# tyshiwo1/Accelerating-T2I-AR-with-SJD

Hardware: AMD Instinct MI355X
Metric: accepted image-tokens/s (SJD, Lumina-mGPT-7B 768px); tokens_per_step = 1/steps-to-converge rate (higher is better)
Workload: dtype bf16; 1 GPU; Lumina-mGPT-7B 768x768, 1 prompt/GPU, draft window 16, CFG 3.0 (batch 2), top-k 2000, bf16, random-init synthetic weights (embed_token_scale=0.7); prompt_len=64, kv_len_start=401, kv_len_end=2064, lead_in_steps=131, prompts=1, parallelism=prompt-parallel x1

## Files before the change

accelerating-t2i-ar-with-sjd_amd/_lib.py:

```python
import ctypes
import os

MAX_WINDOW = 64
MAX_RANGES = 4
DTYPE_BF16, DTYPE_F16, DTYPE_F32 = 0, 1, 2
F1_POST_NORM = 0x100
F2_ROPE_TABLE = 0x200
F2_HEAD_PAD128 = 0x400
K1_HEAD_DIM_100 = 0x800
F2_ONE_HEAD = 0x1000
QKN_SHARDS_SHIFT = 16

_HERE = os.path.dirname(os.path.abspath(__file__))
SO_PATH = os.environ.get("SJD_HIP_LIB") or os.path.join(_HERE, "libsjd_hip.so")


class RowRule(ctypes.Structure):
    _fields_ = [("n_ranges", ctypes.c_int32), ("lo", ctypes.c_int32 * MAX_RANGES), ("hi", ctypes.c_int32 * MAX_RANGES),
                ("forced", ctypes.c_int32), ("top_k", ctypes.c_int32), ("top_p_thr", ctypes.c_float), ("temperature", ctypes.c_float)]


class IterParams(ctypes.Structure):
    _fields_ = [("n_rows", ctypes.c_int32), ("kv_len", ctypes.c_int32), ("use_cfg", ctypes.c_int32),
                ("scheme", ctypes.c_int32), ("n_fresh", ctypes.c_int32), ("batch_rows", ctypes.c_int32), ("iter_seq", ctypes.c_int32), ("philox_blocks", ctypes.c_int32),
                ("philox_seed", ctypes.c_uint64), ("philox_offset", ctypes.c_uint64 * 3),
                ("fresh_tok", ctypes.c_int64 * MAX_WINDOW), ("rules", RowRule * MAX_WINDOW),
                ("resid_rules", RowRule * MAX_WINDOW)]


class State(ctypes.Structure):
    _fields_ = [("m", ctypes.c_int32), ("rejected", ctypes.c_int32), ("n_prev", ctypes.c_int32),
                ("prob_buf", ctypes.c_int32), ("tokens", ctypes.c_int64 * MAX_WINDOW),
                ("win_tok", ctypes.c_int64 * MAX_WINDOW), ("q_src", ctypes.c_int32 * MAX_WINDOW), ("amax", ctypes.c_int64 * MAX_WINDOW)]


class RowNorm(ctypes.Structure):
    _fields_ = [("sumsq", ctypes.c_void_p), ("slices", ctypes.c_int32), ("hidden", ctypes.c_int32), ("eps", ctypes.c_float)]


class RawUnits(ctypes.Structure):
    _fields_ = [("records", ctypes.c_void_p), ("index", ctypes.c_void_p), ("n", ctypes.c_int32)]


class Slots(ctypes.Structure):
    _fields_ = [("n_slots", ctypes.c_int32), ("head_rows", ctypes.c_int32), ("params_stride", ctypes.c_int64), ("state_stride", ctypes.c_int64),
                ("probs_stride", ctypes.c_int64), ("zero_state_stride", ctypes.c_int64), ("scratch_stride", ctypes.c_int64),
                ("mirror_stride", ctypes.c_int64), ("dbg_stride", ctypes.c_int64)]


class HeadPartials(ctypes.Structure):
    _fields_ = [("part", ctypes.c_void_p), ("n_chunks", ctypes.c_int32), ("chunk_stride", ctypes.c_int64), ("row_stride", ctypes.c_int64),
                ("col0", ctypes.c_int32), ("n_cols", ctypes.c_int32), ("urow_off", ctypes.c_int32), ("round_dtype", ctypes.c_int32),
                ("row_sumsq", ctypes.c_void_p), ("slices", ctypes.c_int32), ("prows", ctypes.c_int32), ("inv_hidden", ctypes.c_float),
                ("eps", ctypes.c_float), ("dbg_c", ctypes.c_void_p), ("dbg_u", ctypes.c_void_p), ("zero_state", ctypes.c_void_p)]


class L2Head(ctypes.Structure):
    _fields_ = [("wz", ctypes.c_void_p), ("kind", ctypes.c_int32), ("gx", ctypes.c_int32), ("gy", ctypes.c_int32), ("waves", ctypes.c_int32),
                ("n_tiles", ctypes.c_int32), ("tile0", ctypes.c_int32), ("n_out", ctypes.c_int32), ("pairs_full", ctypes.c_int32),
                ("pairs_last", ctypes.c_int32), ("step_major", ctypes.c_int32), ("head_pairs", ctypes.c_int32)]


EXPORTS = ["sjd_version", "sjd_error_string", "sjd_reguess", "sjd_logits_to_probs_sample", "sjd_verify_accept",
           "sjd_kv_append", "sjd_attention_workspace_bytes", "sjd_draft_window_attention", "sjd_draft_window_attention_ex",
           "sjd_event_create", "sjd_event_destroy", "sjd_event_synchronize", "sjd_event_elapsed_ms",
           "sjd_add_rmsnorm", "sjd_qknorm_rope_append", "sjd_silu_mul", "sjd_gemm_num_chunks", "sjd_skinny_gemm",
           "sjd_kv_append_fp8", "sjd_draft_window_attention_fp8", "sjd_qknorm_rope_append_fp8",
           "sjd_residual_sumsq", "sjd_qknorm_rope_append_ex", "sjd_silu_mul_ex", "sjd_skinny_gemm_cols",
           "sjd_logits_to_probs_sample_part", "sjd_logits_to_probs_sample_ex", "sjd_reguess_ex",
           "sjd_verify_accept_ex", "sjd_upload_async", "sjd_stream_synchronize", "sjd_gateup_silu", "sjd_host_wait_u64",
           "sjd_philox_fill", "sjd_philox_offset_increment", "sjd_skinny_gemm_z", "sjd_gateup_silu_z",
           "sjd_draft_window_attention_colsplit", "sjd_draft_window_attention_fp8_colsplit",
           "sjd_head_combine",
           "sjd_reguess_slots", "sjd_logits_to_probs_sample_part_slots", "sjd_verify_accept_slots",
           "sjd_logits_to_probs_sample_part_slots_g", "sjd_head_combine_g"]
EXP_EXPORTS = ["sjd_weight_prefetch", "sjd_qkv_attention_fused", "sjd_qkv_attention_fused_split", "sjd_skinny_gemm_reduce", "sjd_reduce_timeouts",
               "sjd_draft_window_attention_merged", "sjd_draft_window_attention_fp8_merged", "sjd_mlp_pair_z", "sjd_mlp_pair_timeouts",
               "sjd_l2_head_gemm_z", "sjd_l2_head_gateup_z", "sjd_l2_head_bytes", "sjd_weight_prefetch_head", "sjd_debug_xcc_map", "sjd_residual_sumsq_pf",
               "sjd_skinny_gemm_engine_z", "sjd_engine_timeouts", "sjd_skinny_gemm_wide", "sjd_o_merge_prologue_probe", "sjd_skinny_gemm_z_wide"]
EXP_SO_PATH = os.environ.get("SJD_HIP_EXP_LIB") or os.path.join(_HERE, "libsjd_hip_exp.so")
# ... 120 lines not shown
```

accelerating-t2i-ar-with-sjd_amd/backbones.py:

```python
import math
from dataclasses import dataclass
from typing import Optional

import torch
import torch.nn as nn
import torch.nn.functional as F


import logging as _logging
import os as _os
_log = _logging.getLogger("sjd_amd.backbones")

_K1_FUSED_DEFAULT = _os.environ.get("SJD_K1_FUSED", "0") == "1"
_K1_FUSED_SPLIT_DEFAULT = _os.environ.get("SJD_K1_FUSED_SPLIT", "1") != "0"
_MLP_PAIR_DEFAULT = _os.environ.get("SJD_MLP_PAIR", "0") == "1"
_NAN_CHECK = _os.environ.get("SJD_NAN_CHECK", "0") == "1"


def _chk(tag, x, rows=None):
    if not _NAN_CHECK or x is None:
        return x
    t = x.data if hasattr(x, "n_chunks") else x
    v = t if rows is None else (t[:, :rows] if hasattr(x, "n_chunks") else t[:rows])
    if not torch.isfinite(v.float()).all():
# ... 614 lines not shown
        try:
            self.forward_window(tokens, positions, 0, key_start)
        finally:
            self.cache, attn.params, attn.regime = cache, saved[0], saved[1]
        scales = []
        for li in range(len(self.model.layers)):
            ka = float(tmp.k[li][:, :, :P].abs().amax().float())
            va = float(tmp.v[li][:, :, :P].abs().amax().float())
            scales.append((max(ka, 1e-6) * headroom / 448.0, max(va, 1e-6) * headroom / 448.0))
        attn.layer_scales = scales
        self.buffers_version = getattr(self, "buffers_version", 0) + 1
        return scales

    def _f2(self, qkv, li, qn, pos, B, n, params, kv_len, row_norm=None):
        ops, H, Hkv, D = self._ops, self.n_heads, self.n_kv_heads, self.head_dim
        return ops.qknorm_rope_append(qkv, self.cache.k[li], self.cache.v[li], *qn, self._inv_freq32, pos, B, n, H, Hkv, D, params,
                                      kv_len if params is None else 0, kv_scale=self.attn.scale_of(li) if hasattr(self.attn, "scale_of") else (1.0, 1.0),
                                      dtype=self.lm_head.weight.dtype, row_norm=row_norm, qk_shards=self.args.model_parallel_size)

    def _attention_block(self, qkv_part, li, qn, pos, B, n, params, kv_len, key_start, row_norm=None):
        ops, H, Hkv, D = self._ops, self.n_heads, self.n_kv_heads, self.head_dim
        ks_ok = isinstance(key_start, torch.Tensor) and key_start.is_cuda and key_start.dtype == torch.int32
        if getattr(self, "k1_fused", _K1_FUSED_DEFAULT) and ks_ok and not self.args.swin_norm and self.args.model_parallel_size == 1 and ops.fused_attention_ok(B, n, H, Hkv, D, self.cache.k.dtype):
            ns, ws = 1, None
            if getattr(self, "k1_fused_split", _K1_FUSED_SPLIT_DEFAULT):
                ns = self.attn._resolve_split(B, Hkv, n, H)
                ws = self.attn._workspace(B, H, n, D, self.cache.k.device) if ns > 1 else None
            return ops.qkv_attention_fused(qkv_part, self.cache.k[li], self.cache.v[li], *qn, self._inv_freq32, pos, B, n, H, D, params,
                                           kv_len if params is None else 0, key_start, row_norm=row_norm, dtype=self.lm_head.weight.dtype,
                                           n_split=ns, workspace=ws)
        q = self._f2(qkv_part, li, qn, pos, B, n, params, kv_len, row_norm=row_norm)
        return self.attn.attend(li, q, self.cache, kv_len, key_start)

    def _forward_window_g1_folded(self, tokens, positions, kv_len, key_start, cols=None, head_partials=False):
        ops, B, n = self._ops, tokens.shape[0], tokens.shape[1]
        T, eps, cfg = B * n, self.args.rms_norm_eps, self.G1_CFG
        self._prefetch_plan()
        g1 = lambda x_, name, N_, K_: self._g1(li, x_, name, N_, K_)
        H, Hkv, D, hid, inter = self.n_heads, self.n_kv_heads, self.head_dim, self.args.hidden_size, self.args.intermediate_size
        params = getattr(self.attn, "params", None)
        want_fused = getattr(self, "gateup_fused", _GATEUP_FUSED_DEFAULT)
        fuse_mlp = want_fused and (T <= 64 or want_fused == "tall") and not self._pf_on and ops.gateup_silu_ok(T, inter, hid, cfg["gate_up"][0],
                                                                                                                   isinstance(self._packed[0]["gate_up"], ops.PackedZ))
        red = getattr(self, "reduce_fused", _REDUCE_FUSED_DEFAULT) and not self._pf_on
        raw = lambda name: not isinstance(self._packed[0][name], ops.PackedZ)
        h_dev = self.lm_head.weight.device
        red_o = red and raw("o") and ops.skinny_gemm_reduce_ok(T, hid, H * D, cfg["o"][0], 8, h_dev)
        red_d = red and raw("down") and ops.skinny_gemm_reduce_ok(T, hid, inter, cfg["down"][0], 8, h_dev)
        pair_mlp = (getattr(self, "mlp_pair", _MLP_PAIR_DEFAULT) and fuse_mlp and not red_d and h_dev.type == "cuda" and
                    ops.mlp_pair_ok(T, inter, hid, self._packed[0]["gate_up"], self._packed[0]["down"], cfg["down"][0], cfg["down"][1], h_dev))
        h = self.model.embed_tokens(tokens).view(T, -1).contiguous()
        pos = positions.reshape(T).contiguous()
        delta, ss_next = None, None
        for li, layer in enumerate(self.model.layers):
            a = layer.self_attn
            rn = (ss_next if ss_next is not None else ops.residual_sumsq(h, delta), hid, eps)
            qn = (a.q_norm.weight, a.q_norm.bias, a.k_norm.weight, a.k_norm.bias) if self.args.qk_norm else (None,) * 4
            _chk(f"L{li} sumsq", rn[0][:, :T] if rn[0].dim() == 2 and rn[0].shape[1] >= T else rn[0])
            o = self._attention_block(_chk(f"L{li} qkv", g1(h, "qkv", (H + 2 * Hkv) * D, hid), T), li, qn, pos, B, n, params, kv_len, key_start, row_norm=rn)
            _chk(f"L{li} attention", o)
            if red_o:
                rn = (ops.skinny_gemm_reduce(o.view(T, H * D), self._packed[li]["o"], hid, H * D, cfg["o"][0], h, 8, cfg["o"][2]), hid, eps)
            else:
                rn = (ops.residual_sumsq(h, g1(o.view(T, H * D), "o", hid, H * D)), hid, eps)
            if pair_mlp:
                if getattr(self, "_pair_ready", None) is None or self._pair_ready.device != h.device:
                    self._pair_ready = torch.zeros(max(64, (inter + cfg["down"][0] - 1) // cfg["down"][0] + 1), dtype=torch.int32, device=h.device)
                _, delta = ops.mlp_pair(h, self._packed[li]["gate_up"], self._packed[li]["down"], inter, hid, cfg["down"][0], row_norm=rn,
                                        ready=self._pair_ready)
                ss_next = None
                continue
            if fuse_mlp:
                act = ops.gateup_silu(h, self._packed[li]["gate_up"], inter, hid, cfg["gate_up"][2], row_norm=rn)
            else:
                act = ops.silu_mul(g1(h, "gate_up", 2 * inter, hid), rows=T, dtype=h.dtype, row_norm=rn)
            _chk(f"L{li} act", act)
            if red_d:
                delta, ss_next = None, ops.skinny_gemm_reduce(act, self._packed[li]["down"], hid, inter, cfg["down"][0], h, 8, cfg["down"][2])
            else:
                delta, ss_next = g1(act, "down", hid, inter), None
            _chk(f"L{li} down", delta, T)
            _chk(f"L{li} h", h)
        self._prefetch_join()
        if head_partials and self._packed_head is not None:
            return self._head_partials(h, delta, cols, n, sumsq=ss_next)
        if ss_next is not None:
# ... 5 lines not shown
    def _forward_window_g1(self, tokens, positions, kv_len, key_start, cols=None):
        ops, B, n = self._ops, tokens.shape[0], tokens.shape[1]
        T, eps, cfg = B * n, self.args.rms_norm_eps, self.G1_CFG
        cap = 2560 if T <= 32 else 1 << 30
        if any(c[0] > cap for c in cfg.values()):
            raise ValueError(f"G1_CFG chunk sizes must be <= {cap} for a {T}-row window")
        g1 = lambda x_, name, N_, K_: ops.skinny_gemm(x_, self._packed[li][name], N_, K_, cfg[name][0], cfg[name][1], cfg[name][2])
        H, Hkv, D, hid, inter = self.n_heads, self.n_kv_heads, self.head_dim, self.args.hidden_size, self.args.intermediate_size
        params = getattr(self.attn, "params", None)
        h = self.model.embed_tokens(tokens).view(T, -1).contiguous()
        pos = positions.reshape(T).contiguous()
        delta = None
        swin = self.args.swin_norm
        for li, layer in enumerate(self.model.layers):
            a = layer.self_attn
            x = h if swin else ops.add_rmsnorm(h, delta, layer.input_layernorm.weight, eps)
            qkv = g1(x, "qkv", (H + 2 * Hkv) * D, hid)
            qn = (a.q_norm.weight, a.q_norm.bias, a.k_norm.weight, a.k_norm.bias) if self.args.qk_norm else (None,) * 4
            o = self._attention_block(qkv, li, qn, pos, B, n, params, kv_len, key_start)
            attn_out = g1(o.view(T, H * D), "o", hid, H * D)
            if swin:
                x = ops.add_rmsnorm_post(h, attn_out, layer.input_layernorm.weight, eps)
            else:
                x = ops.add_rmsnorm(h, attn_out, layer.post_attention_layernorm.weight, eps)
            gu = g1(x, "gate_up", 2 * inter, hid)
            act = ops.silu_mul(gu, rows=T, dtype=h.dtype)
            delta = g1(act, "down", hid, inter)
            if swin:
                ops.add_rmsnorm_post(h, delta, layer.post_attention_layernorm.weight, eps)
                delta = None
        x = ops.add_rmsnorm(h, delta, self.model.norm.weight, eps)
        return _head_logits(self.lm_head, x, cols).view(B, n, -1)

    def _forward_window_fused(self, tokens, positions, kv_len, key_start, cols=None, head_partials=False):
        T_ = tokens.shape[0] * tokens.shape[1]
        if self._gemm == "sjd" and (T_ <= 64 or (T_ <= 128 and tokens.shape[1] <= 32) or
                                    (T_ <= 256 and tokens.shape[1] <= 32 and self._packed and not isinstance(self._packed[0]["qkv"], self._ops.PackedZ)
                                     and all(c[1] in self.G1_WIDE_TILES for c in self.G1_CFG.values()))):
            if self._fold_norm:
                return self._forward_window_g1_folded(tokens, positions, kv_len, key_start, cols, head_partials)
            return self._forward_window_g1(tokens, positions, kv_len, key_start, cols)
        ops, B, n = self._ops, tokens.shape[0], tokens.shape[1]
        T, eps = B * n, self.args.rms_norm_eps
        H, Hkv, D = self.n_heads, self.n_kv_heads, self.head_dim
        params = getattr(self.attn, "params", None)
        h = self.model.embed_tokens(tokens).view(T, -1).contiguous()
        pos = positions.reshape(T).contiguous()
        delta = None
        swin = self.args.swin_norm
        for li, layer in enumerate(self.model.layers):
            a = layer.self_attn
            qkv_w, gu_w = self._fused[li]
            x = h if swin else ops.add_rmsnorm(h, delta, layer.input_layernorm.weight, eps)
            qkv = F.linear(x, qkv_w)
            qn = (a.q_norm.weight, a.q_norm.bias, a.k_norm.weight, a.k_norm.bias) if self.args.qk_norm else (None,) * 4
            q = _chk(f"prefill L{li} q", self._f2(_chk(f"prefill L{li} qkv", qkv), li, qn, pos, B, n, params, kv_len))
            o = _chk(f"prefill L{li} attention", self.attn.attend(li, q, self.cache, kv_len, key_start))
            attn_out = F.linear(o.view(T, H * D), a.o_proj.weight)
            if swin:
                x = _chk(f"prefill L{li} norm1", ops.add_rmsnorm_post(h, attn_out, layer.input_layernorm.weight, eps))
                ops.add_rmsnorm_post(h, _chk(f"prefill L{li} mlp", F.linear(ops.silu_mul(F.linear(x, gu_w)), layer.mlp.down_proj.weight)),
                                     layer.post_attention_layernorm.weight, eps)
                continue
            x = _chk(f"prefill L{li} norm2", ops.add_rmsnorm(h, attn_out, layer.post_attention_layernorm.weight, eps))
            delta = _chk(f"prefill L{li} mlp", F.linear(ops.silu_mul(F.linear(x, gu_w)), layer.mlp.down_proj.weight))
        x = ops.add_rmsnorm(h, delta, self.model.norm.weight, eps)
        return _head_logits(self.lm_head, x, cols).view(B, n, -1)

    def forward_window(self, tokens, positions, kv_len, key_start, cols=None, head_partials=False):
        if getattr(self, "_ops", None) is not None:
            return self._forward_window_fused(tokens, positions, kv_len, key_start, cols, head_partials)
        B, n = tokens.shape
        h = self.model.embed_tokens(tokens)
        cos, sin = self._rope(positions, h.dtype)
        for li, layer in enumerate(self.model.layers):
            a = layer.self_attn
            x = h if self.args.swin_norm else layer.input_layernorm(h)
            q = a.q_proj(x).view(B, n, a.num_heads, a.head_dim)
            k = a.k_proj(x).view(B, n, a.num_kv, a.head_dim)
            v = a.v_proj(x).view(B, n, a.num_kv, a.head_dim)
            if self.args.qk_norm:
                q, k = a.q_norm(q), a.k_norm(k)
            q = q * cos + _rotate_half(q) * sin
            k = k * cos + _rotate_half(k) * sin
            o = self.attn(li, q, k, v, self.cache, kv_len, key_start)
            if self.args.swin_norm:
                h = h + layer.input_layernorm(a.o_proj(o.reshape(B, n, -1)))
                h = h + layer.post_attention_layernorm(layer.mlp(h))
                continue
            h = h + a.o_proj(o.reshape(B, n, -1))
            h = h + layer.mlp(layer.post_attention_layernorm(h))
        return _head_logits(self.lm_head, self.model.norm(h), cols)


LUMINA_7B = ChameleonArgs()
CHAMELEON_30B = ChameleonArgs(vocab_size=65536, hidden_size=8192, intermediate_size=22016, num_hidden_layers=48, num_attention_heads=64,
                              num_key_value_heads=8, model_parallel_size=4, swin_norm=True)
EMU3_8B = ChameleonArgs(vocab_size=184622, hidden_size=4096, intermediate_size=14336, num_hidden_layers=32,
                        num_attention_heads=32, num_key_value_heads=8, rms_norm_eps=1e-5, rope_theta=1000000.0,
                        qk_norm=False, max_position_embeddings=9216)
LLAMAGEN_B = LlamaGenArgs(dim=768, n_layer=12, n_head=12)
```

accelerating-t2i-ar-with-sjd_amd/csrc/sjd_sampling.hip:

```cpp
#include <hip/hip_runtime.h>
#include <math.h>
#include <type_traits>

#include "../../include/sjd_hip.h"
#include "sjd_device.h"
#include "sjd_philox.h"

#ifdef SJD_TRACE
__device__ unsigned long long g_k2_trace[64][16];
#define SJD_TRS(slot, i) do { if (threadIdx.x == 0) g_k2_trace[(slot) & 63][i] = wall_clock64(); } while (0)
extern "C" int sjd_debug_trace_k2(unsigned long long *host_out, int n)
{
    return hipMemcpyFromSymbol(host_out, HIP_SYMBOL(g_k2_trace), (size_t)n * 16 * sizeof(unsigned long long), 0, hipMemcpyDeviceToHost) == hipSuccess ? 0 : -1;
}
#else
#define SJD_TRS(slot, i) do { } while (0)
#endif

__device__ __forceinline__ void rule_window(const sjd_row_rule &r, int V, int &lo, int &hi)
{
    if (r.n_ranges == 0) { lo = 0; hi = V; return; }
    lo = V; hi = 0;
#pragma unroll
    for (int a = 0; a < SJD_MAX_RANGES; ++a)
        if (a < r.n_ranges) { lo = min(lo, r.lo[a]); hi = max(hi, r.hi[a]); }
    lo = max(lo, 0); hi = min(hi, V);
    if (hi < lo) hi = lo;
}

__device__ __forceinline__ bool rule_allows(const sjd_row_rule &r, int c)
{
    if (r.n_ranges == 0) return true;
    bool ok = false;
#pragma unroll
    for (int a = 0; a < SJD_MAX_RANGES; ++a) ok |= (a < r.n_ranges) && (c >= r.lo[a]) && (c < r.hi[a]);
    return ok;
}

static_assert(sizeof(sjd_row_rule) == 52 && sizeof(sjd_iter_params) == 64 + 8 * SJD_MAX_WINDOW + 2 * 52 * SJD_MAX_WINDOW, "sjd_iter_params layout is mirrored by ctypes (sjd_amd/_lib.py::IterParams)");
static_assert(sizeof(sjd_head_partials) == 96, "sjd_head_partials layout is mirrored by ctypes (sjd_amd/_lib.py::HeadPartials)");

__device__ __forceinline__ float k2_round16(float x, int dt)
{
    if (dt == SJD_DTYPE_BF16) {
        unsigned u = __float_as_uint(x);
        u += 0x7fffu + ((u >> 16) & 1u);
        return __uint_as_float(u & 0xffff0000u);
    }
    if (dt == SJD_DTYPE_F16) return (float)((_Float16)x);
    return x;
}

__device__ __forceinline__ float k2_row_scale(const sjd_head_partials &hp, int tok)
{
    if (!hp.row_sumsq) return 1.0f;
    float t = 0.f;
    for (int s0 = 0; s0 < hp.slices; s0 += 8) {
        float v[8];
#pragma unroll
        for (int q = 0; q < 8; ++q) v[q] = (s0 + q < hp.slices) ? hp.row_sumsq[(size_t)(s0 + q) * hp.prows + tok] : 0.f;
#pragma unroll
        for (int q = 0; q < 8; ++q) t += v[q];
    }
    return rsqrtf(t * hp.inv_hidden + hp.eps);
}

__device__ __forceinline__ void k2_row_scales(const sjd_head_partials &hp, int tok, float &rc, float &ru)
{
    if (!hp.row_sumsq) return;
    const bool two = hp.urow_off > 0;
    float t = 0.f, tu = 0.f;
    for (int s0 = 0; s0 < hp.slices; s0 += 8) {
// ... 683 lines not shown
                            const unsigned long long cand = pack_vi(dv / sjd_philox_exponential(ph_seed, ph_off2, ph_T2, (uint64_t)col), col);
                            best = cand > best ? cand : best;
                        }
                    } else {
                        SJD_FOR_OWNED_COLS_IN(wlo, whi, c0) {
#pragma unroll
                            for (int j = 0; j < 4; ++j) {
                                const int col = c0 + j;
                                if (col >= wlo && col < whi) {
                                    const float dv = scratch[col - sb] / S;
                                    if (dv > 0.0f) {
                                        const unsigned long long cand = pack_vi(dv / sjd_philox_exponential(ph_seed, ph_off2, ph_T2, (uint64_t)col), col);
                                        best = cand > best ? cand : best;
                                    }
                                }
                            }
                        }
                    }
                }
                SJD_TRS(32, 4);
                const int tok = block_argmax(best, sh);
                if (threadIdx.x == 0) state->tokens[row] = tok;
            }
            };
            if (res_lds) resample(std::true_type{}); else resample(std::false_type{});
        }
    }
    if (threadIdx.x == 0) { state->m = m; state->rejected = rejected ? (degenerate ? 2 : 1) : 0; state->n_prev = n; }
    SJD_TRS(32, 5);
    k4_mirror_state(state, host_mirror, params->iter_seq);
    SJD_TRS(32, 6);
}

template <bool SLOTS = false>
__global__ void k5_reguess(const sjd_iter_params *__restrict__ params, sjd_state *__restrict__ state,
                           int64_t *__restrict__ input_ids_out, int n_batch, int max_rows, const int64_t *__restrict__ pos_offset,
                           int64_t *__restrict__ positions_out, const sjd_slots sb)
{
    if constexpr (SLOTS) {
        const size_t s = blockIdx.x;
        params = reinterpret_cast<const sjd_iter_params *>(reinterpret_cast<const char *>(params) + s * (size_t)sb.params_stride);
        state = reinterpret_cast<sjd_state *>(reinterpret_cast<char *>(state) + s * (size_t)sb.state_stride);
        input_ids_out += s * (size_t)n_batch * (size_t)max_rows;
        if (pos_offset) pos_offset += s * (size_t)n_batch;
        if (positions_out) positions_out += s * (size_t)n_batch * (size_t)max_rows;
    }
    const int i = threadIdx.x;
    const int n = params->n_rows;
    const int m = state->m, n_prev = state->n_prev;
    int a = n_prev - m;
    if (a > n - 1) a = n - 1;
    if (a < 0) a = 0;
    int64_t tok = 0;
    int qs = -1;
    if (i < n) {
        if (i <= a) { tok = state->tokens[m - 1 + i]; qs = m - 1 + i; }
        else { tok = params->fresh_tok[i - 1 - a]; qs = -1; }
    }
    __syncthreads();
    if (i < max_rows) {
        if (i >= n) { tok = state->tokens[m - 1]; qs = -1; }
        state->win_tok[i] = tok;
        state->q_src[i] = qs;
        for (int b = 0; b < n_batch; ++b) input_ids_out[(size_t)b * max_rows + i] = tok;
        if (positions_out) {
            const int64_t base = (int64_t)params->kv_len + i;
            for (int b = 0; b < n_batch; ++b) positions_out[(size_t)b * max_rows + i] = base + (pos_offset ? pos_offset[b] : 0);
        }
    }
}

#define SJD_DRAW_LIST 2304
static int sjd_stage_lds_floats(long cols)
{
    const long cap = 150 * 1024 / 4;
    return (int)(cols < cap ? ((cols + 3) & ~3L) : cap);
}

extern "C" int sjd_reguess_ex(const sjd_iter_params *params, sjd_state *state, int64_t *input_ids_out, int n_batch, int max_rows,
                              const int64_t *pos_offset, int64_t *positions_out, void *stream)
{
    if (!params || !state || !input_ids_out || max_rows < 1 || max_rows > SJD_MAX_WINDOW || n_batch < 1) return SJD_ERR_BAD_ARG;
    hipLaunchKernelGGL(k5_reguess<false>, dim3(1), dim3(64), 0, (hipStream_t)stream, params, state, input_ids_out, n_batch, max_rows, pos_offset,
                       positions_out, sjd_slots{});
    return hipGetLastError() == hipSuccess ? SJD_OK : SJD_ERR_LAUNCH;
}

extern "C" int sjd_reguess(const sjd_iter_params *params, sjd_state *state, int64_t *input_ids_out, int n_batch,
                           int max_rows, void *stream)
{
    return sjd_reguess_ex(params, state, input_ids_out, n_batch, max_rows, nullptr, nullptr, stream);
}

extern "C" int sjd_logits_to_probs_sample_ex(const float *logits_c, const float *logits_u, int64_t row_stride, float guidance,
                                             int max_rows, int V, const sjd_iter_params *params, const float *noise,
                                             float *probs_out, int64_t *tokens_out, int64_t *amax_out, void *stream);

extern "C" int sjd_logits_to_probs_sample(const float *logits_c, const float *logits_u, int64_t row_stride, float guidance,
                                          int max_rows, int V, const sjd_iter_params *params, const float *noise,
                                          float *probs_out, int64_t *tokens_out, void *stream)
{
    return sjd_logits_to_probs_sample_ex(logits_c, logits_u, row_stride, guidance, max_rows, V, params, noise, probs_out, tokens_out, nullptr, stream);
// ... 51 lines not shown
    if (!guidance || ((uintptr_t)guidance & 3)) return SJD_ERR_BAD_ARG;
    return sjd_head_combine_launch(head, 0.0f, guidance, max_rows, V, params, z_out, stream);
}

extern "C" int sjd_verify_accept_ex(const sjd_iter_params *params, sjd_state *state, const float *probs, const float *prev_probs,
                                    const float *rs, const float *noise2, float *scratch, int max_rows, int V, sjd_state *host_mirror,
                                    void *stream)
{
    if (!params || !state || !probs || !prev_probs || !scratch || max_rows < 1 || max_rows > SJD_MAX_WINDOW || V < 1)
        return SJD_ERR_BAD_ARG;
    const int lds_floats = sjd_stage_lds_floats((long)V + 2 * SJD_DRAW_LIST);
    (void)hipFuncSetAttribute((const void *)k4_verify_accept<false>, hipFuncAttributeMaxDynamicSharedMemorySize, lds_floats * 4);
    hipLaunchKernelGGL(k4_verify_accept<false>, dim3(1), dim3(SJD_TPB), (size_t)lds_floats * 4, (hipStream_t)stream, params, state, probs, prev_probs, rs,
                       noise2, scratch, V, host_mirror, lds_floats, sjd_slots{});
    return hipGetLastError() == hipSuccess ? SJD_OK : SJD_ERR_LAUNCH;
}

extern "C" int sjd_verify_accept(const sjd_iter_params *params, sjd_state *state, const float *probs, const float *prev_probs,
                                 const float *rs, const float *noise2, float *scratch, int max_rows, int V, void *stream)
{
    return sjd_verify_accept_ex(params, state, probs, prev_probs, rs, noise2, scratch, max_rows, V, nullptr, stream);
}

static bool sjd_slots_ok(const sjd_slots *sl)
{
    return sl && sl->n_slots >= 1 && sl->n_slots <= 65535 && sl->params_stride >= (int64_t)sizeof(sjd_iter_params) && (sl->params_stride % 8) == 0 &&
           sl->state_stride >= (int64_t)sizeof(sjd_state) && (sl->state_stride % 8) == 0;
}

extern "C" int sjd_reguess_slots(const sjd_iter_params *params0, sjd_state *state0, int64_t *input_ids_out, int n_batch, int max_rows,
                                 const int64_t *pos_offset, int64_t *positions_out, const sjd_slots *slots, void *stream)
{
    if (!params0 || !state0 || !input_ids_out || max_rows < 1 || max_rows > SJD_MAX_WINDOW || n_batch < 1 || !sjd_slots_ok(slots)) return SJD_ERR_BAD_ARG;
    hipLaunchKernelGGL(k5_reguess<true>, dim3(slots->n_slots), dim3(64), 0, (hipStream_t)stream, params0, state0, input_ids_out, n_batch, max_rows,
                       pos_offset, positions_out, *slots);
    return hipGetLastError() == hipSuccess ? SJD_OK : SJD_ERR_LAUNCH;
}

static int sjd_k2_slots_launch(const sjd_head_partials *head, float guidance, const float *guidance_slots, int max_rows, int V,
                               const sjd_iter_params *params0, float *probs_out0, int64_t *tokens_out0, int64_t *amax_out0, const sjd_slots *slots,
                               void *stream)
{
    if (!head || !head->part || head->n_chunks < 1 || head->n_cols < 1 || head->col0 < 0 || head->row_stride < head->n_cols) return SJD_ERR_BAD_ARG;
    if (!params0 || !probs_out0 || !tokens_out0 || max_rows < 1 || max_rows > SJD_MAX_WINDOW || V < 1) return SJD_ERR_BAD_ARG;
    if (head->row_sumsq && (head->slices < 1 || head->prows < 1)) return SJD_ERR_BAD_ARG;
    if (!sjd_slots_ok(slots) || slots->head_rows < max_rows || slots->probs_stride < (int64_t)max_rows * V) return SJD_ERR_BAD_ARG;
    if (head->zero_state && slots->zero_state_stride < 2 * (int64_t)max_rows) return SJD_ERR_BAD_ARG;
    if ((head->dbg_c || head->dbg_u) && slots->dbg_stride < (int64_t)max_rows * V) return SJD_ERR_BAD_ARG;
    const int lds_floats = sjd_stage_lds_floats((long)head->n_cols + 8 + 2 * SJD_DRAW_LIST);
    (void)hipFuncSetAttribute((const void *)k2_logits_to_probs_sample<true, true>, hipFuncAttributeMaxDynamicSharedMemorySize, lds_floats * 4);
    hipLaunchKernelGGL((k2_logits_to_probs_sample<true, true>), dim3(max_rows, slots->n_slots), dim3(SJD_TPB), (size_t)lds_floats * 4, (hipStream_t)stream,
                       (const float *)nullptr, (const float *)nullptr, (long)0, guidance, V, params0, (const float *)nullptr, probs_out0, tokens_out0, *head,
                       amax_out0, lds_floats, *slots, guidance_slots);
    return hipGetLastError() == hipSuccess ? SJD_OK : SJD_ERR_LAUNCH;
}

extern "C" int sjd_logits_to_probs_sample_part_slots(const sjd_head_partials *head, float guidance, int max_rows, int V, const sjd_iter_params *params0,
                                                     float *probs_out0, int64_t *tokens_out0, int64_t *amax_out0, const sjd_slots *slots, void *stream)
{
    return sjd_k2_slots_launch(head, guidance, nullptr, max_rows, V, params0, probs_out0, tokens_out0, amax_out0, slots, stream);
}

extern "C" int sjd_logits_to_probs_sample_part_slots_g(const sjd_head_partials *head, const float *guidance, int max_rows, int V,
                                                       const sjd_iter_params *params0, float *probs_out0, int64_t *tokens_out0, int64_t *amax_out0,
                                                       const sjd_slots *slots, void *stream)
{
// ... 37 lines not shown
```

accelerating-t2i-ar-with-sjd_amd/engine.py:

```python
import contextlib
import ctypes
import gc
import os
import random
import time
import warnings
from dataclasses import dataclass, field
from typing import List, Optional

import numpy as np
import torch

from . import _lib as L
from . import ops
from .grammar import spatial_fresh_tokens


_MIRROR_STREAM_WAIT = os.environ.get("SJD_MIRROR_SPIN", "0") != "1"
_TWO_STAGE = os.environ.get("SJD_TWO_STAGE", "0") == "1"


@dataclass
class SJDConfig:
    jacobi_loop_interval_l: int = 1
# ... 147 lines not shown
        p = self.params.view
        p.n_rows, p.kv_len, p.use_cfg, p.scheme, p.n_fresh = n, kv_len, int(use_cfg), scheme, len(fresh)
        self._seq = (self._seq % 0x7FFFFFF0) + 1
        p.iter_seq = self._seq
        if philox is None:
            p.philox_blocks = 0
        else:
            p.philox_blocks, p.philox_seed = philox[0], philox[1]
            p.philox_offset[0], p.philox_offset[1], p.philox_offset[2] = philox[2], philox[3], philox[4]
        if fresh:
            p.fresh_tok[:len(fresh)] = fresh
        self._write_rules(L.IterParams.rules.offset, rules)
        if resid:
            self._write_rules(L.IterParams.resid_rules.offset, resid)
        self.params.upload(L.IterParams.resid_rules.offset if head_only else None)

    def _write_rules(self, offset, rules):
        key = tuple(map(id, rules))
        blk = self._rule_bytes.get(key)
        if blk is None:
            blk = b"".join(bytes(r) for r in rules)
            if len(self._rule_bytes) < 4096:
                self._rule_bytes[key] = blk
                self._rule_keep.append(list(rules))
        ctypes.memmove(self.params.host.data_ptr() + offset, blk, len(blk))

    def _upload_resid(self, resid):
        off = L.IterParams.resid_rules.offset
        self._write_rules(off, resid)
        L.check(L.load().sjd_upload_async(self.params.dev.data_ptr() + off, self.params.host.data_ptr() + off, self.params.nbytes - off,
                                          ops._stream()), "sjd_upload_async")

    def _forward_body(self, cols=None):
        ops.reguess(self.params, self.state, self.input_ids, pos_offset=self.pos_offset, positions_out=self.positions)
        positions = self.positions
        if self.head_partials:
            return self.backbone.forward_window(self.input_ids, positions, -1, self.key_start, cols=cols, head_partials=True)
        if cols is None:
            return self.backbone.forward_window(self.input_ids, positions, -1, self.key_start)
        return self.backbone.forward_window(self.input_ids, positions, -1, self.key_start, cols=cols)

    def _calibrate_fp8(self, tokens, positions, key_start):
        bb = self.backbone
        cache, attn = getattr(bb, "cache", None), getattr(bb, "attn", None)
        if (cache is None or cache.k.dtype != ops.FP8 or attn is None or getattr(attn, "layer_scales", 1) is not None
                or getattr(attn, "kv_scale", (1.0, 1.0)) != (1.0, 1.0) or not hasattr(bb, "calibrate_kv_scales")
                or os.environ.get("SJD_FP8_CALIBRATE", "1") == "0"):
            return
        bb.calibrate_kv_scales(tokens, positions, key_start)

    def _k2_out(self):
        return (self.amax_ptr, self.tokens_ptr) if getattr(self, "_greedy", False) else (self.tokens_ptr, self.amax_ptr)

    def _sample_body(self, cur, logits, cols=None):
        noise, rs, noise2 = (None, None, None) if self._philox else (self.noise, self.rs, self.noise2[0])
        if isinstance(logits, ops.HeadOut):
            dbg = None
            if self.hook is not None:
                if self._dbg is None:
                    self._dbg = torch.zeros(2, self.Lmax, self.V, dtype=torch.float32, device=self.device)
                dbg = self._dbg
                dbg.zero_()
            tok_out, amax_out = self._k2_out()
            ops.logits_to_probs_sample_part(logits, self._guidance, self.params, noise, self.probs[cur], tok_out, dbg=dbg,
                                            amax_out_ptr=amax_out, zero_state=self.zero_state[cur])
        else:
            lu = logits[1] if self.B > 1 else None
            tok_out, amax_out = self._k2_out()
# ... 316 lines not shown
```

accelerating-t2i-ar-with-sjd_amd/ops.py:

```python
import ctypes
import os

import torch

from . import _lib as L


def _stream():
    return ctypes.c_void_p(torch.cuda.current_stream().cuda_stream)


def _ptr(t):
    return ctypes.c_void_p(0 if t is None else t.data_ptr())


def _dtype_code(dt):
    if dt == torch.bfloat16:
        return L.DTYPE_BF16
    if dt == torch.float16:
        return L.DTYPE_F16
    if dt == torch.float32:
        return L.DTYPE_F32
    raise L.SjdLibraryError(f"SJD HIP kernels support bf16/fp16 KV and activations, got {dt}")

# ... 103 lines not shown
            st = self.nbytes + 8
            self._mirrors = torch.zeros(len(self.blobs) * st, dtype=torch.uint8, pin_memory=True)
            for i, b in enumerate(self.blobs):
                b._mirror = self._mirrors[i * st:(i + 1) * st]
        return ctypes.c_void_p(self._mirrors.data_ptr()), self.nbytes + 8

    def upload(self):
        L.check(L.load().sjd_upload_async(self.dev.data_ptr(), self.host.data_ptr(), self.host.numel(), _stream()), "sjd_upload_async")

    def download(self):
        self.host.copy_(self.dev)

    def wait_mirror(self):
        L.check(L.load().sjd_stream_synchronize(_stream()), "sjd_stream_synchronize")
        for b in self.blobs:
            if b._mirror is not None:
                b.collect_mirror()

    @property
    def ptr(self):
        return ctypes.c_void_p(self.dev.data_ptr())


def reguess(params: DeviceBlob, state: DeviceBlob, input_ids_out: torch.Tensor, pos_offset=None, positions_out=None):
    n_batch, max_rows = input_ids_out.shape
    assert input_ids_out.dtype == torch.int64 and input_ids_out.is_contiguous()
    if positions_out is None:
        L.check(L.load().sjd_reguess(params.ptr, state.ptr, _ptr(input_ids_out), n_batch, max_rows, _stream()), "sjd_reguess")
        return
    assert positions_out.dtype == torch.int64 and positions_out.is_contiguous() and tuple(positions_out.shape) == (n_batch, max_rows)
    assert pos_offset is None or (pos_offset.dtype == torch.int64 and pos_offset.is_contiguous() and pos_offset.numel() == n_batch)
    L.check(L.load().sjd_reguess_ex(params.ptr, state.ptr, _ptr(input_ids_out), n_batch, max_rows, _ptr(pos_offset) if pos_offset is not None else None,
                                   _ptr(positions_out), _stream()), "sjd_reguess_ex")


def logits_to_probs_sample(logits_c, logits_u, guidance, params: DeviceBlob, noise, probs_out, tokens_out_ptr, col0=0, amax_out_ptr=None):
    max_rows, V = probs_out.shape
    assert logits_c.dtype == torch.float32 and logits_c.stride(-1) == 1 and probs_out.is_contiguous()
    assert noise is None or (noise.dtype == torch.float32 and noise.is_contiguous() and noise.shape[-1] == V)
    if logits_u is not None:
        assert logits_u.stride(-2) == logits_c.stride(-2) and logits_u.stride(-1) == 1
    shift = lambda t: ctypes.c_void_p(0 if t is None else t.data_ptr() - 4 * int(col0))
    L.check(L.load().sjd_logits_to_probs_sample_ex(shift(logits_c), shift(logits_u), logits_c.stride(-2), float(guidance),
                                                  max_rows, V, params.ptr, _ptr(noise), _ptr(probs_out), tokens_out_ptr, amax_out_ptr,
                                                  _stream()), "sjd_logits_to_probs_sample")


def verify_accept(params: DeviceBlob, state: DeviceBlob, probs, prev_probs, rs, noise2, scratch, mirror=False):
    max_rows, V = probs.shape
    for t in (probs, prev_probs, rs, noise2, scratch):
        assert t is None or (t.dtype == torch.float32 and t.is_contiguous())
    L.check(L.load().sjd_verify_accept_ex(params.ptr, state.ptr, _ptr(probs), _ptr(prev_probs), _ptr(rs), _ptr(noise2),
                                         _ptr(scratch), max_rows, V, state.mirror_ptr if mirror else None, _stream()), "sjd_verify_accept")


def kv_append(k_new, v_new, k_cache, v_cache, params, kv_len):
    B, n, Hkv, D = k_new.shape
    assert k_new.is_contiguous() and v_new.is_contiguous() and k_cache.is_contiguous() and v_cache.is_contiguous()
    L.check(L.load().sjd_kv_append(_ptr(k_new), _ptr(v_new), _ptr(k_cache), _ptr(v_cache), B, n, Hkv, D,
                                  k_cache.shape[2], _dtype_code(k_new.dtype), params.ptr if params is not None else None,
                                  int(kv_len), _stream()), "sjd_kv_append")


FP8 = torch.float8_e4m3fn


# ... 847 lines not shown
```

include/sjd_hip.h:

```cpp
#ifndef SJD_HIP_H
#define SJD_HIP_H

#include <stdint.h>

#ifdef __cplusplus
extern "C" {
#endif

#define SJD_VERSION 104
#define SJD_MAX_WINDOW 64
#define SJD_MAX_RANGES 4

#define SJD_OK 0
#define SJD_ERR_BAD_ARG (-1)
#define SJD_ERR_UNSUPPORTED (-2)
#define SJD_ERR_LAUNCH (-3)

#define SJD_DTYPE_BF16 0
#define SJD_DTYPE_F16 1
#define SJD_DTYPE_F32 2

#define SJD_DTYPE_MASK 0xff
#define SJD_F1_POST_NORM 0x100
#define SJD_F2_ROPE_TABLE 0x200
// ... 77 lines not shown
                               int max_rows, int V, const sjd_iter_params *params, const float *noise,
                               float *probs_out, int64_t *tokens_out, void *stream);
int sjd_logits_to_probs_sample_ex(const float *logits_c, const float *logits_u, int64_t row_stride, float guidance,
                                  int max_rows, int V, const sjd_iter_params *params, const float *noise,
                                  float *probs_out, int64_t *tokens_out, int64_t *amax_out, void *stream);

typedef struct sjd_head_partials {
    const float *part;
    int32_t n_chunks;
    int64_t chunk_stride;
    int64_t row_stride;
    int32_t col0, n_cols;
    int32_t urow_off;
    int32_t round_dtype;
    const float *row_sumsq;
    int32_t slices, prows;
    float inv_hidden, eps;
    float *dbg_c, *dbg_u;
    int32_t *zero_state;
} sjd_head_partials;
int sjd_logits_to_probs_sample_part(const sjd_head_partials *head , float guidance,
                                    int max_rows, int V, const sjd_iter_params *params, const float *noise, float *probs_out,
                                    int64_t *tokens_out, int64_t *amax_out , void *stream);

int sjd_head_combine(const sjd_head_partials *head , float guidance, int max_rows, int V,
                     const sjd_iter_params *params, float *z_out, void *stream);

int sjd_head_combine_g(const sjd_head_partials *head, const float *guidance , int max_rows, int V, const sjd_iter_params *params,
                       float *z_out, void *stream);

int sjd_verify_accept(const sjd_iter_params *params, sjd_state *state, const float *probs, const float *prev_probs,
                      const float *rs, const float *noise2, float *scratch, int max_rows, int V, void *stream);

typedef struct sjd_slots {
    int32_t n_slots;
    int32_t head_rows;
    int64_t params_stride;
    int64_t state_stride;
    int64_t probs_stride;
    int64_t zero_state_stride;
    int64_t scratch_stride;
    int64_t mirror_stride;
    int64_t dbg_stride;
} sjd_slots;
int sjd_reguess_slots(const sjd_iter_params *params0, sjd_state *state0, int64_t *input_ids_out, int n_batch, int max_rows,
                      const int64_t *pos_offset, int64_t *positions_out, const sjd_slots *slots, void *stream);
int sjd_logits_to_probs_sample_part_slots(const sjd_head_partials *head, float guidance, int max_rows, int V, const sjd_iter_params *params0,
                                          float *probs_out0, int64_t *tokens_out0, int64_t *amax_out0 , const sjd_slots *slots,
                                          void *stream);
int sjd_logits_to_probs_sample_part_slots_g(const sjd_head_partials *head, const float *guidance, int max_rows, int V, const sjd_iter_params *params0,
                                            float *probs_out0, int64_t *tokens_out0, int64_t *amax_out0 , const sjd_slots *slots,
                                            void *stream);
int sjd_verify_accept_slots(const sjd_iter_params *params0, sjd_state *state0, const float *probs0, const float *prev_probs0, float *scratch0,
                            int max_rows, int V, sjd_state *host_mirror0 , const sjd_slots *slots, void *stream);

int sjd_kv_append(const void *k_new, const void *v_new, void *k_cache, void *v_cache, int B, int n_rows, int H_kv,
                  int D, int S_max, int dtype, const sjd_iter_params *params, int kv_len, void *stream);

int64_t sjd_attention_workspace_bytes(int B, int H, int n_rows, int D, int n_split);
int sjd_draft_window_attention(const void *q, const void *k_cache, const void *v_cache, void *out, int B, int n_rows,
                               int H, int H_kv, int D, int S_max, int dtype, const int32_t *key_start,
                               const sjd_iter_params *params, int kv_len, int n_split, void *workspace, void *stream);

int sjd_draft_window_attention_ex(const void *q, const void *k_cache, const void *v_cache, void *out, int B, int n_rows,
                                  int H, int H_kv, int D, int S_max, int dtype, const int32_t *key_start,
                                  const sjd_iter_params *params, int kv_len, int n_split, void *workspace, void *stream,
                                  void *ev_start, void *ev_stop);



int sjd_add_rmsnorm(void *h, const void *delta, const void *weight, void *y, int rows, int hidden, float eps, int dtype,
                    const float *part, int n_chunks, void *stream);
int sjd_qknorm_rope_append(const void *qkv, void *q_out, void *k_cache, void *v_cache, const void *qn_w, const void *qn_b,
                           const void *kn_w, const void *kn_b, const float *inv_freq, const int64_t *positions, int B, int n,
                           int H, int H_kv, int D, int S_max, int dtype, const sjd_iter_params *params, int kv_len,
                           const float *part, int n_chunks, void *stream);
// ... 77 lines not shown
```

Measured before the change: 767.1 image-tokens/s.

## Fuse window reguess with embedding gather and first-layer row sum-of-squares

Adds a kernel that builds the draft window's token ids and positions, gathers their embedding rows, and computes per-slice row sum-of-squares in one launch. The folded-norm G1 forward then starts from these embedded rows and the precomputed sumsq instead of running the embedding lookup and the first residual_sumsq. This removes two small launches plus a read of the hidden state per step, at the cost of a new ctypes struct field in sjd_slots and a path that only applies when T<=64 with the sjd GEMM and norm folding.

```diff
diff --git a/accelerating-t2i-ar-with-sjd_amd/_lib.py b/accelerating-t2i-ar-with-sjd_amd/_lib.py
--- a/accelerating-t2i-ar-with-sjd_amd/_lib.py
+++ b/accelerating-t2i-ar-with-sjd_amd/_lib.py
@@ -42,10 +42,15 @@
     _fields_ = [("records", ctypes.c_void_p), ("index", ctypes.c_void_p), ("n", ctypes.c_int32)]
 
 
+class WindowHead(ctypes.Structure):
+    _fields_ = [("embed", ctypes.c_void_p), ("h_out", ctypes.c_void_p), ("sumsq_out", ctypes.c_void_p), ("vocab", ctypes.c_int32),
+                ("hidden", ctypes.c_int32), ("dtype", ctypes.c_int32), ("reserved", ctypes.c_int32)]
+
+
 class Slots(ctypes.Structure):
     _fields_ = [("n_slots", ctypes.c_int32), ("head_rows", ctypes.c_int32), ("params_stride", ctypes.c_int64), ("state_stride", ctypes.c_int64),
                 ("probs_stride", ctypes.c_int64), ("zero_state_stride", ctypes.c_int64), ("scratch_stride", ctypes.c_int64),
-                ("mirror_stride", ctypes.c_int64), ("dbg_stride", ctypes.c_int64)]
+                ("mirror_stride", ctypes.c_int64), ("dbg_stride", ctypes.c_int64), ("window_head", ctypes.POINTER(WindowHead))]
 
 
 class HeadPartials(ctypes.Structure):
diff --git a/accelerating-t2i-ar-with-sjd_amd/backbones.py b/accelerating-t2i-ar-with-sjd_amd/backbones.py
--- a/accelerating-t2i-ar-with-sjd_amd/backbones.py
+++ b/accelerating-t2i-ar-with-sjd_amd/backbones.py
@@ -670,7 +670,15 @@
         q = self._f2(qkv_part, li, qn, pos, B, n, params, kv_len, row_norm=row_norm)
         return self.attn.attend(li, q, self.cache, kv_len, key_start)
 
-    def _forward_window_g1_folded(self, tokens, positions, kv_len, key_start, cols=None, head_partials=False):
+    def window_head_ok(self, T):
+        w = self.model.embed_tokens.weight
+        return (getattr(self, "_ops", None) is not None and self._gemm == "sjd" and self._fold_norm and T <= 64 and w.is_cuda and w.is_contiguous()
+                and w.dtype in (torch.bfloat16, torch.float16))
+
+    def window_head(self, params, state, input_ids_out, pos_offset, positions_out):
+        return self._ops.reguess_embed_sumsq(params, state, input_ids_out, pos_offset, positions_out, self.model.embed_tokens.weight)
+
+    def _forward_window_g1_folded(self, tokens, positions, kv_len, key_start, cols=None, head_partials=False, embedded=None):
         ops, B, n = self._ops, tokens.shape[0], tokens.shape[1]
         T, eps, cfg = B * n, self.args.rms_norm_eps, self.G1_CFG
         self._prefetch_plan()
@@ -687,9 +695,13 @@
         red_d = red and raw("down") and ops.skinny_gemm_reduce_ok(T, hid, inter, cfg["down"][0], 8, h_dev)
         pair_mlp = (getattr(self, "mlp_pair", _MLP_PAIR_DEFAULT) and fuse_mlp and not red_d and h_dev.type == "cuda" and
                     ops.mlp_pair_ok(T, inter, hid, self._packed[0]["gate_up"], self._packed[0]["down"], cfg["down"][0], cfg["down"][1], h_dev))
-        h = self.model.embed_tokens(tokens).view(T, -1).contiguous()
+        delta, ss_next = None, None
+        if embedded is not None:
+            h, ss_next = embedded
+            assert tuple(h.shape) == (T, hid) and h.is_contiguous()
+        else:
+            h = self.model.embed_tokens(tokens).view(T, -1).contiguous()
         pos = positions.reshape(T).contiguous()
-        delta, ss_next = None, None
         for li, layer in enumerate(self.model.layers):
             a = layer.self_attn
             rn = (ss_next if ss_next is not None else ops.residual_sumsq(h, delta), hid, eps)
@@ -761,13 +773,15 @@
         x = ops.add_rmsnorm(h, delta, self.model.norm.weight, eps)
         return _head_logits(self.lm_head, x, cols).view(B, n, -1)
 
-    def _forward_window_fused(self, tokens, positions, kv_len, key_start, cols=None, head_partials=False):
+    def _forward_window_fused(self, tokens, positions, kv_len, key_start, cols=None, head_partials=False, embedded=None):
         T_ = tokens.shape[0] * tokens.shape[1]
+        if embedded is not None and not self.window_head_ok(T_):
+            raise ValueError("forward_window(embedded=...): only the folded-norm G1 window forward starts from window_head()'s output")
         if self._gemm == "sjd" and (T_ <= 64 or (T_ <= 128 and tokens.shape[1] <= 32) or
                                     (T_ <= 256 and tokens.shape[1] <= 32 and self._packed and not isinstance(self._packed[0]["qkv"], self._ops.PackedZ)
                                      and all(c[1] in self.G1_WIDE_TILES for c in self.G1_CFG.values()))):
             if self._fold_norm:
-                return self._forward_window_g1_folded(tokens, positions, kv_len, key_start, cols, head_partials)
+                return self._forward_window_g1_folded(tokens, positions, kv_len, key_start, cols, head_partials, embedded)
             return self._forward_window_g1(tokens, positions, kv_len, key_start, cols)
         ops, B, n = self._ops, tokens.shape[0], tokens.shape[1]
         T, eps = B * n, self.args.rms_norm_eps
@@ -796,9 +810,11 @@
         x = ops.add_rmsnorm(h, delta, self.model.norm.weight, eps)
         return _head_logits(self.lm_head, x, cols).view(B, n, -1)
 
-    def forward_window(self, tokens, positions, kv_len, key_start, cols=None, head_partials=False):
+    def forward_window(self, tokens, positions, kv_len, key_start, cols=None, head_partials=False, embedded=None):
         if getattr(self, "_ops", None) is not None:
-            return self._forward_window_fused(tokens, positions, kv_len, key_start, cols, head_partials)
+            return self._forward_window_fused(tokens, positions, kv_len, key_start, cols, head_partials, embedded)
+        if embedded is not None:
+            raise ValueError("forward_window(embedded=...) needs the fused path (enable_fused)")
         B, n = tokens.shape
         h = self.model.embed_tokens(tokens)
         cos, sin = self._rope(positions, h.dtype)
diff --git a/accelerating-t2i-ar-with-sjd_amd/csrc/sjd_sampling.hip b/accelerating-t2i-ar-with-sjd_amd/csrc/sjd_sampling.hip
--- a/accelerating-t2i-ar-with-sjd_amd/csrc/sjd_sampling.hip
+++ b/accelerating-t2i-ar-with-sjd_amd/csrc/sjd_sampling.hip
@@ -5,6 +5,7 @@
 #include "../../include/sjd_hip.h"
 #include "sjd_device.h"
 #include "sjd_philox.h"
+#include "sjd_mlp_epilogue.h"
 
 #ifdef SJD_TRACE
 __device__ unsigned long long g_k2_trace[64][16];
@@ -38,6 +39,7 @@
 }
 
 static_assert(sizeof(sjd_row_rule) == 52 && sizeof(sjd_iter_params) == 64 + 8 * SJD_MAX_WINDOW + 2 * 52 * SJD_MAX_WINDOW, "sjd_iter_params layout is mirrored by ctypes (sjd_amd/_lib.py::IterParams)");
+static_assert(sizeof(sjd_window_head) == 40 && sizeof(sjd_slots) == 72 && offsetof(sjd_slots, window_head) == 64, "sjd_slots / sjd_window_head layouts are mirrored by ctypes (sjd_amd/_lib.py::Slots, WindowHead)");
 static_assert(sizeof(sjd_head_partials) == 96, "sjd_head_partials layout is mirrored by ctypes (sjd_amd/_lib.py::HeadPartials)");
 
 __device__ __forceinline__ float k2_round16(float x, int dt)
@@ -787,6 +789,19 @@
     SJD_TRS(32, 6);
 }
 
+__device__ __forceinline__ void k5_window_row(const sjd_iter_params *__restrict__ params, const sjd_state *__restrict__ state, int i,
+                                              int64_t &tok, int &qs)
+{
+    const int n = params->n_rows;
+    const int m = state->m, n_prev = state->n_prev;
+    int a = n_prev - m;
+    if (a > n - 1) a = n - 1;
+    if (a < 0) a = 0;
+    if (i >= n) { tok = state->tokens[m - 1]; qs = -1; }
+    else if (i <= a) { tok = state->tokens[m - 1 + i]; qs = m - 1 + i; }
+    else { tok = params->fresh_tok[i - 1 - a]; qs = -1; }
+}
+
 template <bool SLOTS = false>
 __global__ void k5_reguess(const sjd_iter_params *__restrict__ params, sjd_state *__restrict__ state,
                            int64_t *__restrict__ input_ids_out, int n_batch, int max_rows, const int64_t *__restrict__ pos_offset,
@@ -801,20 +816,11 @@
         if (positions_out) positions_out += s * (size_t)n_batch * (size_t)max_rows;
     }
     const int i = threadIdx.x;
-    const int n = params->n_rows;
-    const int m = state->m, n_prev = state->n_prev;
-    int a = n_prev - m;
-    if (a > n - 1) a = n - 1;
-    if (a < 0) a = 0;
     int64_t tok = 0;
     int qs = -1;
-    if (i < n) {
-        if (i <= a) { tok = state->tokens[m - 1 + i]; qs = m - 1 + i; }
-        else { tok = params->fresh_tok[i - 1 - a]; qs = -1; }
-    }
+    if (i < max_rows) k5_window_row(params, state, i, tok, qs);
     __syncthreads();
     if (i < max_rows) {
-        if (i >= n) { tok = state->tokens[m - 1]; qs = -1; }
         state->win_tok[i] = tok;
         state->q_src[i] = qs;
         for (int b = 0; b < n_batch; ++b) input_ids_out[(size_t)b * max_rows + i] = tok;
@@ -823,6 +829,49 @@
             for (int b = 0; b < n_batch; ++b) positions_out[(size_t)b * max_rows + i] = base + (pos_offset ? pos_offset[b] : 0);
         }
     }
+}
+
+__device__ __forceinline__ float k5e_wave_sum(float v)
+{
+#pragma unroll
+    for (int off = 32; off >= 1; off >>= 1) v += __shfl_xor(v, off);
+    return v;
+}
+
+template <int DT>
+__global__ __launch_bounds__(128) void k5e_reguess_embed_sumsq(const sjd_iter_params *__restrict__ params, sjd_state *__restrict__ state,
+                                                               int64_t *__restrict__ input_ids_out, int n_batch, int max_rows,
+                                                               const int64_t *__restrict__ pos_offset, int64_t *__restrict__ positions_out,
+                                                               const unsigned short *__restrict__ embed, int vocab, int hidden,
+                                                               unsigned short *__restrict__ h_out, float *__restrict__ out_sumsq, int prows,
+                                                               long params_stride, long state_stride)
+{
+    __shared__ float red[2];
+    const int row = blockIdx.x, i = row % max_rows, sb = row / max_rows;
+    const size_t s = (size_t)(sb / n_batch);
+    params = reinterpret_cast<const sjd_iter_params *>(reinterpret_cast<const char *>(params) + s * (size_t)params_stride);
+    state = reinterpret_cast<sjd_state *>(reinterpret_cast<char *>(state) + s * (size_t)state_stride);
+    int64_t tok;
+    int qs;
+    k5_window_row(params, state, i, tok, qs);
+    if (blockIdx.y == 0 && threadIdx.x == 0) {
+        input_ids_out[row] = tok;
+        if (positions_out) positions_out[row] = (int64_t)params->kv_len + i + (pos_offset ? pos_offset[sb] : 0);
+        if (sb % n_batch == 0) { state->win_tok[i] = tok; state->q_src[i] = qs; }
+    }
+    const int64_t trow = tok < 0 ? 0 : (tok >= vocab ? vocab - 1 : tok);
+    const int c = blockIdx.y * 512 + threadIdx.x * 4;
+    float ss = 0.f;
+    if (c < hidden) {
+        const uint2 hv = *reinterpret_cast<const uint2 *>(embed + (size_t)trow * hidden + c);
+        *reinterpret_cast<uint2 *>(h_out + (size_t)row * hidden + c) = hv;
+        ss = sjd_sumsq4(ss, SjdAct<DT>::to_f((unsigned short)(hv.x & 0xffffu)), SjdAct<DT>::to_f((unsigned short)(hv.x >> 16)),
+                        SjdAct<DT>::to_f((unsigned short)(hv.y & 0xffffu)), SjdAct<DT>::to_f((unsigned short)(hv.y >> 16)));
+    }
+    ss = k5e_wave_sum(ss);
+    if ((threadIdx.x & 63) == 0) red[threadIdx.x >> 6] = ss;
+    __syncthreads();
+    if (threadIdx.x == 0) out_sumsq[(size_t)blockIdx.y * prows + row] = red[0] + red[1];
 }
 
 #define SJD_DRAW_LIST 2304
@@ -940,6 +989,19 @@
                                  const int64_t *pos_offset, int64_t *positions_out, const sjd_slots *slots, void *stream)
 {
     if (!params0 || !state0 || !input_ids_out || max_rows < 1 || max_rows > SJD_MAX_WINDOW || n_batch < 1 || !sjd_slots_ok(slots)) return SJD_ERR_BAD_ARG;
+    if (const sjd_window_head *wh = slots->window_head) {
+        const long rows = (long)slots->n_slots * n_batch * max_rows;
+        if (!wh->embed || !wh->h_out || !wh->sumsq_out || wh->vocab < 1 || wh->hidden < 4 || (wh->hidden % 4) != 0 || rows > 256 ||
+            ((uintptr_t)wh->embed & 7) || ((uintptr_t)wh->h_out & 7)) return SJD_ERR_BAD_ARG;
+        if (wh->dtype != SJD_DTYPE_BF16 && wh->dtype != SJD_DTYPE_F16) return SJD_ERR_UNSUPPORTED;
+        const int prows = (((int)rows + 31) / 32) * 32;
+        const dim3 grid((unsigned)rows, (wh->hidden + 511) / 512), block(128);
+        auto kern = wh->dtype == SJD_DTYPE_BF16 ? k5e_reguess_embed_sumsq<SJD_DTYPE_BF16> : k5e_reguess_embed_sumsq<SJD_DTYPE_F16>;
+        hipLaunchKernelGGL(kern, grid, block, 0, (hipStream_t)stream, params0, state0, input_ids_out, n_batch, max_rows, pos_offset, positions_out,
+                           (const unsigned short *)wh->embed, wh->vocab, wh->hidden, (unsigned short *)wh->h_out, wh->sumsq_out, prows,
+                           (long)slots->params_stride, (long)slots->state_stride);
+        return hipGetLastError() == hipSuccess ? SJD_OK : SJD_ERR_LAUNCH;
+    }
     hipLaunchKernelGGL(k5_reguess<true>, dim3(slots->n_slots), dim3(64), 0, (hipStream_t)stream, params0, state0, input_ids_out, n_batch, max_rows,
                        pos_offset, positions_out, *slots);
     return hipGetLastError() == hipSuccess ? SJD_OK : SJD_ERR_LAUNCH;
diff --git a/accelerating-t2i-ar-with-sjd_amd/engine.py b/accelerating-t2i-ar-with-sjd_amd/engine.py
--- a/accelerating-t2i-ar-with-sjd_amd/engine.py
+++ b/accelerating-t2i-ar-with-sjd_amd/engine.py
@@ -203,8 +203,15 @@
                                           ops._stream()), "sjd_upload_async")
 
     def _forward_body(self, cols=None):
-        ops.reguess(self.params, self.state, self.input_ids, pos_offset=self.pos_offset, positions_out=self.positions)
         positions = self.positions
+        head_ok = getattr(self.backbone, "window_head_ok", None)
+        if head_ok is not None and head_ok(self.B * self.Lmax):
+            embedded = self.backbone.window_head(self.params, self.state, self.input_ids, self.pos_offset, positions)
+            kw = dict(cols=cols, embedded=embedded)
+            if self.head_partials:
+                kw["head_partials"] = True
+            return self.backbone.forward_window(self.input_ids, positions, -1, self.key_start, **kw)
+        ops.reguess(self.params, self.state, self.input_ids, pos_offset=self.pos_offset, positions_out=positions)
         if self.head_partials:
             return self.backbone.forward_window(self.input_ids, positions, -1, self.key_start, cols=cols, head_partials=True)
         if cols is None:
diff --git a/accelerating-t2i-ar-with-sjd_amd/ops.py b/accelerating-t2i-ar-with-sjd_amd/ops.py
--- a/accelerating-t2i-ar-with-sjd_amd/ops.py
+++ b/accelerating-t2i-ar-with-sjd_amd/ops.py
@@ -159,6 +159,30 @@
     assert pos_offset is None or (pos_offset.dtype == torch.int64 and pos_offset.is_contiguous() and pos_offset.numel() == n_batch)
     L.check(L.load().sjd_reguess_ex(params.ptr, state.ptr, _ptr(input_ids_out), n_batch, max_rows, _ptr(pos_offset) if pos_offset is not None else None,
                                    _ptr(positions_out), _stream()), "sjd_reguess_ex")
+
+
+def reguess_embed_sumsq(params, state, input_ids_out, pos_offset, positions_out, embed, h_out=None, sumsq_out=None):
+    n_slots = len(params.blobs) if isinstance(params, BlobArray) else 1
+    B, max_rows = input_ids_out.shape
+    assert B % n_slots == 0 and input_ids_out.dtype == torch.int64 and input_ids_out.is_contiguous()
+    assert positions_out is None or (positions_out.dtype == torch.int64 and positions_out.is_contiguous() and tuple(positions_out.shape) == (B, max_rows))
+    assert pos_offset is None or (pos_offset.dtype == torch.int64 and pos_offset.is_contiguous() and pos_offset.numel() == B)
+    assert embed.dim() == 2 and embed.is_contiguous() and embed.device == input_ids_out.device
+    vocab, hidden = embed.shape
+    T = B * max_rows
+    if h_out is None:
+        h_out = torch.empty(T, hidden, dtype=embed.dtype, device=embed.device)
+    if sumsq_out is None:
+        sumsq_out = torch.empty((hidden + 511) // 512, _prows(T), dtype=torch.float32, device=embed.device)
+    assert h_out.is_contiguous() and h_out.dtype == embed.dtype and tuple(h_out.shape) == (T, hidden)
+    assert sumsq_out.is_contiguous() and sumsq_out.dtype == torch.float32 and tuple(sumsq_out.shape) == ((hidden + 511) // 512, _prows(T))
+    wh = L.WindowHead(embed.data_ptr(), h_out.data_ptr(), sumsq_out.data_ptr(), vocab, hidden, _dtype_code(embed.dtype), 0)
+    sl = L.Slots()
+    sl.n_slots, sl.params_stride, sl.state_stride = n_slots, params.nbytes, state.nbytes
+    sl.window_head = ctypes.pointer(wh)
+    L.check(L.load().sjd_reguess_slots(params.ptr, state.ptr, _ptr(input_ids_out), B // n_slots, max_rows, _ptr(pos_offset), _ptr(positions_out),
+                                      ctypes.byref(sl), _stream()), "sjd_reguess_slots (window head)")
+    return h_out, sumsq_out
 
 
 def logits_to_probs_sample(logits_c, logits_u, guidance, params: DeviceBlob, noise, probs_out, tokens_out_ptr, col0=0, amax_out_ptr=None):
diff --git a/include/sjd_hip.h b/include/sjd_hip.h
--- a/include/sjd_hip.h
+++ b/include/sjd_hip.h
@@ -133,6 +133,16 @@
 int sjd_verify_accept(const sjd_iter_params *params, sjd_state *state, const float *probs, const float *prev_probs,
                       const float *rs, const float *noise2, float *scratch, int max_rows, int V, void *stream);
 
+typedef struct sjd_window_head {
+    const void *embed;
+    void *h_out;
+    float *sumsq_out;
+    int32_t vocab;
+    int32_t hidden;
+    int32_t dtype;
+    int32_t reserved;
+} sjd_window_head;
+
 typedef struct sjd_slots {
     int32_t n_slots;
     int32_t head_rows;
@@ -143,6 +153,7 @@
     int64_t scratch_stride;
     int64_t mirror_stride;
     int64_t dbg_stride;
+    const sjd_window_head *window_head;
 } sjd_slots;
 int sjd_reguess_slots(const sjd_iter_params *params0, sjd_state *state0, int64_t *input_ids_out, int n_batch, int max_rows,
                       const int64_t *pos_offset, int64_t *positions_out, const sjd_slots *slots, void *stream);
```

Result: no change. 765.4 image-tokens/s (-0.2%).
